# dmalyuta/explicit_hybrid_mpc

Measured on AMD Instinct MI355X. Metric: oracle LP solves/sec + final regions/sec, 4-state 2-input N=5 hybrid MPC, higher is better.
Workload: dtype f64

## Files before the change

explicit_hybrid_mpc_amd/csrc/ehm_dev.h:

```cpp
#pragma once

#include <hip/hip_runtime.h>
#include <stdint.h>

namespace ehm {

struct DevProblem {
    int n, m, p, n_u, n_delta;
    const double* Gt;
    const double* St;
    const double* w;
    const double* c;
    double eps_a, eps_r;
    const double* Wc2;
    int lda2, ncw2;
    const double* Wc4;
    int lda4, ncw4, tot4;
    int nd0, LE4;
    int wc_lds;
    const double* Wr3;
    int mpad3;
    const double* Hq;
    const double* Fq;
    const double* f0q;
// ... 78 lines not shown
        b1 = fmin(b1a, b1b);
        if (b1 < thr) return b1;
    }
    const int npairs = nr * (nr - 1) / 2;
    for (int t = lane; t < npairs; t += 64) {
        int a = 0, rem = t;
        while (rem >= nr - 1 - a) {
            rem -= nr - 1 - a;
            ++a;
        }
        const int c = a + 1 + rem;
        const double* fa = scr + a * na;
        const double* fc = scr + c * na;
        double m = -1e300;
        bool ok = true;
        for (int j = 0; j < na; ++j) {
            ok = ok && (fa[j] == fa[j]) && (fc[j] == fc[j]);
            m = fmax(m, fmin(fa[j], fc[j]));
        }
        for (int u = 0; u < na; ++u)
            for (int v = u + 1; v < na; ++v) {
                const double du = fa[u] - fc[u], dv = fa[v] - fc[v];
                if (du * dv < 0.0) {
                    const double den = du - dv;
                    double rc = __builtin_amdgcn_rcp(den);
                    rc = fma(rc, fma(-den, rc, 1.0), rc);
                    rc = fma(rc, fma(-den, rc, 1.0), rc);
                    const double sx = du * rc;
                    m = fmax(m, fma(sx, fa[v] - fa[u], fa[u]));
                }
            }
        if (ok) b = fmin(b, m);
    }
#define EHM_DPP_MIN_STEP(CTRL, RMASK)                                                          \
    {                                                                                          \
        const int lo = __builtin_amdgcn_update_dpp(__double2loint(1e300), __double2loint(b),   \
                                                   CTRL, RMASK, 0xf, false);                   \
        const int hi = __builtin_amdgcn_update_dpp(__double2hiint(1e300), __double2hiint(b),   \
                                                   CTRL, RMASK, 0xf, false);                   \
        b = fmin(b, __hiloint2double(hi, lo));                                                 \
    }
    EHM_DPP_MIN_STEP(0x111, 0xf)
    EHM_DPP_MIN_STEP(0x112, 0xf)
    EHM_DPP_MIN_STEP(0x114, 0xf)
    EHM_DPP_MIN_STEP(0x118, 0xf)
    EHM_DPP_MIN_STEP(0x142, 0xa)
    EHM_DPP_MIN_STEP(0x143, 0xc)
#undef EHM_DPP_MIN_STEP
    const int lo = __builtin_amdgcn_readlane(__double2loint(b), 63);
    const int hi = __builtin_amdgcn_readlane(__double2hiint(b), 63);
    return __hiloint2double(hi, lo);
}

struct DevCounters {
    unsigned long long lp_solves;
    unsigned long long ipm_iters;
    unsigned long long stalled;
    unsigned long long min_margin_bits;
    unsigned long long errors;
    unsigned long long slack_solves;
    unsigned long long slack_iters;
    unsigned long long cert_closed;
    unsigned long long wit_open;
    unsigned long long routed;
    unsigned long long wit_inherited;
    unsigned long long mid_shared;
    unsigned long long wit_table;
    unsigned long long prof[10];
    unsigned long long phase[24];
    unsigned int ticket;
    unsigned int ticket_pad;
};

__host__ __device__ inline int rec_off_vcost(int p) { return (p + 1) * p; }
__host__ __device__ inline int rec_off_vinput(int p) { return (p + 1) * p + (p + 1); }
__host__ __device__ inline int rec_doubles(int p, int n_u) {
    return (p + 1) * p + (p + 1) + (p + 1) * n_u;
}

enum { LP_POINT = 0, LP_FEAS = 1, LP_MIN_SIMPLEX = 2, LP_SLACK = 3, LP_FEAS_SIMPLEX = 4 };
enum { SX_MIN = 0, SX_SLACK = 1, SX_FEAS = 2 };

__host__ __device__ inline int lp_cols(const DevProblem& P, int kind) {
    switch (kind) {
        case LP_POINT: return P.n;
        case LP_FEAS: return P.n + 1;
        case LP_MIN_SIMPLEX: return P.n + P.p;
        case LP_FEAS_SIMPLEX: return P.n + P.p + 1;
        default: return P.n + P.p + 1;
    }
}
__host__ __device__ inline int lp_rows(const DevProblem& P, int kind) {
    switch (kind) {
        case LP_POINT: return P.m;
        case LP_FEAS: return P.m + 1;
        case LP_MIN_SIMPLEX: return P.m + P.p + 1;
        case LP_FEAS_SIMPLEX: return P.m + P.p + 2;
        default: return P.m + P.p + 3;
    }
}

__device__ inline void longest_edge(const double* R, int p, int& bi, int& bj) {
#pragma clang fp contract(off)
    double best = -1.0;
    bi = 0;
    bj = 1;
// ... 54 lines not shown
```

explicit_hybrid_mpc_amd/csrc/ehm_k2.h:

```cpp
#pragma once

#include <hip/hip_runtime.h>
#include <stdint.h>

#include "ehm_dev.h"

#ifndef EHM_K2_THREADS
#define EHM_K2_THREADS 768
#endif

#define K2_AUG_MIN 32
#define K2_HOT_GRAD 176
#define EHM_ROUTE_TOL 1e-6
#define EHM_REQUEUED 0x40000000

namespace ehm {

__host__ __device__ inline size_t k2_node_doubles(int p, int n_u) {
    const size_t nrec = ((size_t)rec_doubles(p, n_u) + 7) & ~(size_t)7;
    const size_t aug = (2 * (size_t)p * p > K2_AUG_MIN) ? 2 * (size_t)p * p : K2_AUG_MIN;
    return (nrec + aug + (size_t)p * p + 8 + 1) & ~(size_t)1;
}

__host__ __device__ inline int k2_stash_doubles(int p, int n_u) {
    return (n_u + 2 * p + 2 + 1) & ~1;
}

__host__ __device__ inline int lp_xbase(int m, int ne) {
    if (ne == 0) return m;
    const int r = m & 63;
    return (r != 0 && r + ne <= 64) ? m : ((m + 63) & ~63);
}
__host__ __device__ inline int lp_slots(int m, int ne) {
    return (lp_xbase(m, ne) + ne + 63) >> 6;
}

struct PersistCtl {
    int head;
    int pad0[31];
    int tail;
    int pad1[31];
    int pending;
    int pad2[31];
    int n_nodes;
    int pad3[31];
    int abort;
    int max_depth_seen;
    int truncated;
    int pad4;
    unsigned long long closed;
    unsigned long long splits;
    unsigned long long repl_closed, repl_splits, repl_solves;
    unsigned long long pushes;
};

struct PersistDeal {
    int pop_limit;
    int depth, rank, world;
    int mix;
    int keep;
    int check;
    int eager;
};

struct K2Gather {
// ... 54 lines not shown
```

explicit_hybrid_mpc_amd/csrc/ehm_persist.h:

```cpp
#ifndef EHM_PERSIST_H
#define EHM_PERSIST_H

#ifndef kx_persist
#error "kx_persist (the kernel's name) must be defined, and the namespace aliases kd / ke declared"
#endif

#define EHM_PERSIST_WATCHDOG_TICKS (60LL * 100000000LL)
#ifndef EHM_PERSIST_MIDFIRST
#define EHM_PERSIST_MIDFIRST 0
#endif
__global__ __launch_bounds__(EHM_K2_THREADS) void kx_persist(
    DevProblem P, DevTree T, int32_t* slots, int n_slots, PersistCtl* ctl, int node_cap,
    DevCounters* cnt, int wave_doubles, int sign_only, int max_depth, PersistDeal deal) {
    double* sm = reinterpret_cast<double*>(k2_smem);
    const int tid = threadIdx.x;
    const int lane0 = tid & 63;
    const int wave = __builtin_amdgcn_readfirstlane(tid >> 6);
    kd::Shared S;
    kd::carve_shared(S, sm, P);
    ke::Shared Se;
    ke::carve_shared(Se, sm, P);
#if EHM2_PROF
    S.gprof = cnt ? cnt->phase : nullptr;
    Se.gprof = cnt ? cnt->phase : nullptr;
#endif
    kd::NodeBuf nb;
    kd::carve_node(nb, sm + kd::shared_doubles(P) + (size_t)wave * wave_doubles, P.p, P.n_u);
    ke::NodeBuf nbe;
    ke::carve_node(nbe, sm + kd::shared_doubles(P) + (size_t)wave * wave_doubles, P.p, P.n_u);
    const int p = P.p, n_u = P.n_u;
    const int nrec = rec_doubles(p, n_u);
    kd::load_shared(P, 0, sm, tid, blockDim.x);
    __syncthreads();
    const long long t_start = wall_clock64();
    unsigned long long* wst = reinterpret_cast<unsigned long long*>(nb.aug);
    double* wmargin = nb.aug + 16;
    enum { W_SOLVES = 0, W_ITERS, W_STALLED, W_ERRORS, W_SLACK, W_SLACK_ITERS, W_CLOSED, W_SPLITS,
           W_DEPTH, W_TRUNC, W_CERT, W_WIT, W_ROUTED, W_RCLOSED, W_RSPLITS, W_RSOLVES,
           W_INH = 17, W_MT = 18, W_MTPARK = 19,
           W_TQ = 20, W_TMT = 21, W_TMID = 22, W_TSLK = 23, W_NMT = 24,
           W_WITT = 25, W_TPRE = 26, W_TPOST = 27, W_REQ = 28,
           W_EAGER = 29, W_PUSH = 30 };
    if (lane0 < 31 && lane0 != 16) wst[lane0] = 0ULL;
    if (lane0 == 0) *wmargin = 1e300;
    kd::wsync();
    int keep = -1;
    bool hot = false;
    int hot_dep = 0, hot_d = 0;
    bool hot_tested = false;
    const bool keep_child = deal.keep != 0;
    for (;;) {
        int id = -1;
        const bool is_hot = hot && keep >= 0;
        hot = false;
        if (keep >= 0) {
            id = keep;
            keep = -1;
        } else if (lane0 == 0) {
            const int idx = atomicAdd(&ctl->head, 1);
            if (idx < ((deal.pop_limit > 0 && deal.pop_limit < n_slots) ? deal.pop_limit
                                                                        : n_slots)) {
                long long t_q = 0;
                for (;;) {
                    id = __hip_atomic_load(&slots[idx], __ATOMIC_RELAXED, __HIP_MEMORY_SCOPE_AGENT);
                    if (id >= 0) break;
                    if (!t_q) t_q = wall_clock64();
                    if (__hip_atomic_load(&ctl->pending, __ATOMIC_RELAXED,
                                          __HIP_MEMORY_SCOPE_AGENT) <= 0 ||
                        __hip_atomic_load(&ctl->abort, __ATOMIC_RELAXED,
                                          __HIP_MEMORY_SCOPE_AGENT) != 0)
                        break;
                    if (wall_clock64() - t_start > EHM_PERSIST_WATCHDOG_TICKS) {
                        atomicMax(&ctl->abort, 3);
                        break;
                    }
                    __builtin_amdgcn_s_sleep(64);
                }
                if (t_q) wst[W_TQ] += (unsigned long long)(wall_clock64() - t_q);
            }
        }
        id = __builtin_amdgcn_readfirstlane(id);
        if (id < 0) break;
        const bool came_back = (id & EHM_REQUEUED) != 0;
        id &= ~EHM_REQUEUED;
        const long long t_pre = wall_clock64();
        const int lane = kd::pin(lane0);
        double* node = nb.rec;
        double* hgrad = nb.lp + K2_HOT_GRAD;
        const int ng = (p + 1) * p;
        int dep = hot_dep;
        if (!is_hot) {
            __builtin_amdgcn_fence(__ATOMIC_ACQUIRE, "agent");
            const double* rec = T.rec + (size_t)id * T.rec_stride;
            const double g_in = (T.grad && lane < ng) ? T.grad[(size_t)id * ng + lane] : 0.0;
#if EHM_PERSIST_MIDFIRST
            const double w_in = (T.wit && sign_only && lane < p + 2)
                ? T.wit[(size_t)id * (p + 2) + lane] : 0.0;
#endif
            dep = T.depth[id];
            for (int k = lane; k < nrec; k += 64) node[k] = rec[k];
            if (T.grad) {
                if (lane < ng) hgrad[lane] = g_in;
                for (int k = lane + 64; k < ng; k += 64) hgrad[k] = T.grad[(size_t)id * ng + k];
            }
#if EHM_PERSIST_MIDFIRST
            if (T.wit && sign_only && lane < p + 2)
                nb.rec[(size_t)wave_doubles - k2_stash_doubles(p, n_u) + n_u + p + lane] = w_in;
#endif
        }
        kd::wsync();
#if EHM_PERSIST_MIDFIRST
        auto lp_free_verdict = [&](const double* rec_, const double* g_, const double* w_,
                                   bool bound_done, double& tw, double& bnd) -> int {
            bool w_open = false;
            if (T.wit && sign_only) {
                const double* Vc = rec_ + rec_off_vcost(p);
                double vbw = 0.0;
                for (int q = 0; q <= p; ++q) vbw = fma(w_[1 + q], Vc[q], vbw);
                const double cw = w_[0];
                tw = fmin(vbw - cw - P.eps_a, vbw - (1.0 + P.eps_r) * cw);
                w_open = tw > EHM_ROUTE_TOL * (1.0 + fabs(vbw));
            }
            if (!(T.grad && sign_only) || bound_done || (w_open && !deal.check)) return w_open ? 1 : 0;
            const double thr = -EHM_ROUTE_TOL * (1.0 + fabs(rec_[rec_off_vcost(p)]));
            bnd = cut_bound(rec_, g_, p, P.eps_a, P.eps_r, lane, nb.lp, thr);
            if (w_open) {
                if (bnd < thr && lane == 0) wst[W_ERRORS] += 1;
                kd::wsync();
                return 1;
            }
            return bnd < thr ? 2 : 0;
        };
        bool inh_open = false;
        double inh_tw = 0.0;
        {
            double bnd = 0.0;
            const int verdict = lp_free_verdict(
                node, hgrad, nb.rec + (size_t)wave_doubles - k2_stash_doubles(p, n_u) + n_u + p,
                is_hot && hot_tested, inh_tw, bnd);
            inh_open = verdict == 1;
            if (verdict == 2) {
                if (lane == 0) {
                    const int dep0 = dep;
                    wst[W_CERT] += 1;
                    wst[W_CLOSED] += 1;
                    if (dep0 < deal.depth) wst[W_RCLOSED] += 1;
                    *wmargin = fmin(*wmargin, -bnd);
                    if ((unsigned long long)dep0 > wst[W_DEPTH]) wst[W_DEPTH] = (unsigned long long)dep0;
                    T.tstar[id] = bnd;
                    if (is_hot) T.flags[id] = 3;
                    else T.flags[id] |= 1;
                    atomicSub(&ctl->pending, 1);
                }
                kd::wsync();
                continue;
            }
        }
#else
        bool inh_open = false;
        double inh_tw = 0.0;
        if (T.grad && sign_only && inh_open && deal.check) {
            const double thr = -EHM_ROUTE_TOL * (1.0 + fabs(node[rec_off_vcost(p)]));
            const double bnd = cut_bound(node, hgrad, p, P.eps_a, P.eps_r, lane, nb.lp, thr);
            if (bnd < thr && lane == 0) wst[W_ERRORS] += 1;
            kd::wsync();
        }
        if (T.grad && sign_only && !inh_open) {
            const double thr = -EHM_ROUTE_TOL * (1.0 + fabs(node[rec_off_vcost(p)]));
            const double bnd = cut_bound(node, hgrad, p, P.eps_a, P.eps_r, lane, nb.lp, thr);
            if (bnd < thr) {
                if (lane == 0) {
                    const int dep0 = dep;
                    wst[W_CERT] += 1;
                    wst[W_CLOSED] += 1;
                    if (dep0 < deal.depth) wst[W_RCLOSED] += 1;
                    *wmargin = fmin(*wmargin, -bnd);
                    if ((unsigned long long)dep0 > wst[W_DEPTH]) wst[W_DEPTH] = (unsigned long long)dep0;
                    T.tstar[id] = bnd;
// ... 24 lines not shown
        bool decided = false;
        int c0_early = 0;
        bool alloc_early = false;
        if (T.wit && sign_only) {
            if (inh_open) {
                open = true;
                decided = true;
                have_wit = true;
                tst = inh_tw;
                margin = inh_tw;
                if (lane == 0) wst[W_INH] += 1;
            }
        }
        if (can_split) {
            longest_edge_wave(node, p, lane, bi, bj);
            if (lane < p) {
#pragma clang fp contract(off)
                mid[lane] = (node[bi * p + lane] + node[bj * p + lane]) / 2.0;
            }
            kd::wsync();
            if (T.mt.state) {
                unsigned int mt_i = 0u;
                int mt_slot = 0;
                const unsigned long long mt_tg = mt_tag(mid, p, T.mt.mask, &mt_i);
                if (lane == 0) {
                    wst[W_TPRE] += (unsigned long long)(wall_clock64() - t_pre);
                    long long waited = 0;
                    const bool may_requeue = decided && !came_back && deal.pop_limit <= 0 &&
                                             id < EHM_REQUEUED;
                    mt_res = mt_claim(T.mt, mt_tg, mt_i, t_start, EHM_PERSIST_WATCHDOG_TICKS,
                                      &mt_slot, &waited, may_requeue);
                    if (mt_res == MT_BUSY) {
                        const int t = atomicAdd(&ctl->tail, 1);
                        if (t < n_slots) {
                            __hip_atomic_store(&slots[t], id | EHM_REQUEUED, __ATOMIC_RELAXED,
                                               __HIP_MEMORY_SCOPE_AGENT);
                            wst[W_REQ] += 1;
                        } else {
                            mt_res = mt_claim(T.mt, mt_tg, mt_i, t_start,
                                              EHM_PERSIST_WATCHDOG_TICKS, &mt_slot, &waited);
                        }
                    }
                    if (waited) {
                        wst[W_TMT] += (unsigned long long)waited;
                        wst[W_NMT] += 1;
                    }
                }
                mt_res = __builtin_amdgcn_readfirstlane(mt_res);
                mt_slot = __builtin_amdgcn_readfirstlane(mt_slot);
                if (mt_res == MT_BUSY) {
                    kd::wsync();
                    continue;
                }
                if (deal.eager && decided) {
                    alloc_early = true;
                    if (lane == 0) c0_early = atomicAdd(&ctl->n_nodes, 2);
                }
                if (mt_res == MT_HIT) {
                    bool same = false;
                    const double ev = mt_read(T.mt, mt_slot, lane, mid, p, &same);
                    if (!same) {
                        mt_res = MT_NONE;
                    } else {
                        const int word = (int)__shfl(ev, 9);
                        Jm = __shfl(ev, 8);
                        mid_status = word & 0xff;
                        mid_conv = ((word >> 8) & 1) != 0;
                        mid_iters = 0;
                        if (lane >= 10 && lane < 10 + n_u) stash[lane - 10] = ev;
                        if (T.grad && lane >= 18 && lane < 18 + p) stash[st_g + lane - 18] = ev;
                        if (lane == 0) wst[W_MT] += 1;
                    }
                }
                if (lane == 0) wst[W_MTPARK] = (unsigned long long)mt_res |
                                               ((unsigned long long)mt_slot << 2);
            } else if (deal.eager && decided) {
                alloc_early = true;
                if (lane == 0) c0_early = atomicAdd(&ctl->n_nodes, 2);
            }
            if (mt_res != MT_HIT)
            {
            const long long t_mid = wall_clock64();
            ke::Wave Wm;
            ke::IpmResult rm;
            for (int attempt = 0; attempt < EHM2_ATTEMPTS; ++attempt) {
                double b[ke::SLOTS];
                const int ln = kd::pin(lane);
                ke::assemble_point(Se, Wm, nbe.lp, mid, false, b, ln, P, 0);
                rm = ke::ipm_solve(Se, Wm, b, ln, false, ke::step_fraction(attempt),
                                   T.grad ? nb.F : nullptr);
                its += rm.iters;
                if (rm.status == 0) break;
            }
#if EHM2_QUAD
            if (T.grad) ke::quad_grad_add(Wm, P, 0, mid, nb.F, lane);
#endif
            Jm = rm.obj;
            mid_status = rm.status;
            mid_conv = (rm.status == 0) && (rm.merit <= 1.0);
            mid_iters = its;
            if (lane < n_u) stash[lane] = Wm.xb[lane];
            if (lane == 0) wst[W_TMID] += (unsigned long long)(wall_clock64() - t_mid);
            }
            if (mt_res != MT_HIT && T.grad && lane < p) stash[st_g + lane] = nb.F[lane];
            kd::wsync();
            if (T.mt.state) {
                const unsigned long long park = wst[W_MTPARK];
                mt_res = (int)(park & 3ull);
                if (mt_res == MT_OWN) {
                    unsigned int mt_i = 0u;
                    const unsigned long long mt_tg = mt_tag(mid, p, T.mt.mask, &mt_i);
                    mt_publish(T.mt, (int)(park >> 2), mt_tg, lane, mid, p, Jm, mid_status,
                               mid_conv ? 1 : 0, mid_iters, stash, n_u,
                               T.grad ? stash + st_g : nullptr);
                }
            }
            if (sign_only && mid_conv && !decided) {
                const double* Vc = node + rec_off_vcost(p);
                const double vb = 0.5 * (Vc[bi] + Vc[bj]);
                const double tw = fmin(vb - Jm - P.eps_a, vb - (1.0 + P.eps_r) * Jm);
                if (tw > EHM_ROUTE_TOL * (1.0 + fabs(vb))) {
                    open = true;
                    decided = true;
                    tst = tw;
                    margin = tw;
                    if (lane == 0) wst[W_WIT] += 1;
                }
            }
        }
// ... 52 lines not shown
                    kd::wsync();
                }
            }
        }
#endif
        if (!decided) {
            const long long t_slk = wall_clock64();
            kd::Wave W;
            kd::IpmResult r;
            its = 0;
            for (int attempt = 0; attempt < EHM2_ATTEMPTS; ++attempt) {
                double b[kd::SLOTS];
                const int ln = kd::pin(lane);
                kd::assemble_simplex(S, W, nb, node, node + rec_off_vcost(p), SX_SLACK, P.eps_a,
                                     P.eps_r, b, ln, P, 0);
                r = kd::ipm_solve(S, W, b, ln, sign_only != 0, kd::step_fraction(attempt));
                its += r.iters;
                if (r.status == 0) break;
            }
            tst = -r.obj;
            open = (tst >= 0.0);
            margin = r.margin;
            const int slack_status = r.status;
#if !EHM2_QUAD
            if (T.wit && sign_only && open && slack_status == 0) {
                const int nz = S.n;
                double cz = 0.0, sb = 0.0;
                for (int q = 0; q < nz; ++q) cz = fma(S.cv[q], W.xb[kd::zcol(W, S, q)], cz);
                for (int q = 0; q < p; ++q) sb += W.xb[W.psi0 + q];
                kd::wsync();
                if (lane == 0) {
                    wit[0] = fma(EHM_WIT_REL, margin, cz);
                    wit[1] = 1.0 - sb;
                }
                if (lane < p) wit[2 + lane] = W.xb[W.psi0 + lane];
                have_wit = true;
                kd::wsync();
            }
#endif
            if (lane == 0) {
                wst[W_TSLK] += (unsigned long long)(wall_clock64() - t_slk);
                wst[W_SOLVES] += 1;
                if (dep < deal.depth) wst[W_RSOLVES] += 1;
                wst[W_ITERS] += (unsigned long long)its;
                wst[W_SLACK] += 1;
                wst[W_SLACK_ITERS] += (unsigned long long)its;
                if (slack_status != 0) {
                    wst[W_STALLED] += 1;
                    wst[W_ERRORS] += 1;
                    T.flags[id] |= 8;
                }
            }
        }
        if (lane == 0) {
            if (can_split) {
                if (mt_res != MT_HIT) {
                    wst[W_SOLVES] += 1;
                    if (dep < deal.depth) wst[W_RSOLVES] += 1;
                    wst[W_ITERS] += (unsigned long long)mid_iters;
                }
                if (mid_status != 0 && open) {
                    wst[W_STALLED] += 1;
                    wst[W_ERRORS] += 1;
                    T.flags[id] |= 16;
                }
            }
            *wmargin = fmin(*wmargin, margin);
            if (margin < EHM_ROUTE_TOL * (1.0 + fabs(node[rec_off_vcost(p)]))) wst[W_ROUTED] += 1;
            if ((unsigned long long)dep > wst[W_DEPTH]) wst[W_DEPTH] = (unsigned long long)dep;
            T.tstar[id] = tst;
            if (!open) {
                T.flags[id] |= 1;
                wst[W_CLOSED] += 1;
                if (dep < deal.depth) wst[W_RCLOSED] += 1;
            }
        }
        if (!open) {
            if (lane == 0) atomicSub(&ctl->pending, 1);
            kd::wsync();
            continue;
        }
        if (!can_split) {
            if (lane == 0) {
                wst[W_TRUNC] = 1;
                atomicSub(&ctl->pending, 1);
            }
            kd::wsync();
            continue;
        }
        const long long t_post = wall_clock64();
        const bool dealt = deal.world > 1 && dep + 1 == deal.depth;
        const bool fast = keep_child && !dealt;
        const bool eager = deal.eager != 0 && sign_only && T.grad && !dealt;
        const bool stage = fast || eager;
        double* hg0 = nb.lp + 256;
        double* cw0 = nb.lp + 328;
        double* c0rec = nb.lp + 340;
        const double gv0 = (T.grad && lane < ng) ? T.grad[(size_t)id * ng + lane] : 0.0;
        const int d = is_hot ? hot_d : T.didx[id];
        int c0 = c0_early;
        if (!alloc_early && lane == 0) c0 = atomicAdd(&ctl->n_nodes, 2);
        c0 = __builtin_amdgcn_readfirstlane(c0);
        if (c0 + 2 > node_cap) {
            if (lane == 0) {
                atomicMax(&ctl->abort, 1);
                atomicSub(&ctl->pending, 1);
            }
            break;
        }
        struct { double obj; } r = {Jm};
        if (T.grad) {
            const double* gp_ = T.grad + (size_t)id * ng;
            double* g0 = T.grad + (size_t)c0 * ng;
            for (int k = lane; k < ng; k += 64) {
                const double gv = (k < 64) ? gv0 : gp_[k];
                const double a0 = (k >= bi * p && k < bi * p + p) ? stash[st_g + k - bi * p] : gv;
                const double a1 = (k >= bj * p && k < bj * p + p) ? stash[st_g + k - bj * p] : gv;
                __hip_atomic_store(g0 + k, a0, __ATOMIC_RELAXED, __HIP_MEMORY_SCOPE_AGENT);
                __hip_atomic_store(g0 + ng + k, a1, __ATOMIC_RELAXED, __HIP_MEMORY_SCOPE_AGENT);
                if (stage) hgrad[k] = a1;
                if (eager) hg0[k] = a0;
            }
        }
        if (T.wit && lane < p + 2) {
            double* w0 = T.wit + (size_t)c0 * (p + 2);
            double v0 = 0.0, v1 = 0.0;
            if (have_wit) {
                witness_for_children(wit, node + rec_off_vcost(p), bi, bj, lane, v0, v1);
            }
            __hip_atomic_store(w0 + lane, v0, __ATOMIC_RELAXED, __HIP_MEMORY_SCOPE_AGENT);
            __hip_atomic_store(w0 + (p + 2) + lane, v1, __ATOMIC_RELAXED, __HIP_MEMORY_SCOPE_AGENT);
            kd::wsync();
            if (stage) wit[lane] = v1;
            if (eager) cw0[lane] = v0;
        }
        if (lane == 0) {
            wst[W_SPLITS] += 1;
            if (dep < deal.depth) wst[W_RSPLITS] += 1;
        }
        const double* xmid = stash;
#else
        kd::IpmResult r;
        int its = 0;
        {
            kd::Wave W;
            for (int attempt = 0; attempt < EHM2_ATTEMPTS; ++attempt) {
                double b[kd::SLOTS];
                const int ln = kd::pin(lane);
                kd::assemble_simplex(S, W, nb, node, node + rec_off_vcost(p), SX_SLACK, P.eps_a,
                                     P.eps_r, b, ln, P, 0);
                r = kd::ipm_solve(S, W, b, ln, sign_only != 0, kd::step_fraction(attempt));
                its += r.iters;
                if (r.status == 0) break;
            }
        }
        r.iters = its;
        const double tst = -r.obj;
        const bool open = (tst >= 0.0);
        if (lane == 0) {
            wst[W_SOLVES] += 1;
            if (dep < deal.depth) wst[W_RSOLVES] += 1;
            wst[W_ITERS] += (unsigned long long)r.iters;
            wst[W_SLACK] += 1;
            wst[W_SLACK_ITERS] += (unsigned long long)r.iters;
            if (r.status != 0) {
                wst[W_STALLED] += 1;
                wst[W_ERRORS] += 1;
                T.flags[id] |= 8;
            }
            *wmargin = fmin(*wmargin, r.margin);
            if (r.margin < EHM_ROUTE_TOL * (1.0 + fabs(node[rec_off_vcost(p)]))) wst[W_ROUTED] += 1;
            if ((unsigned long long)dep > wst[W_DEPTH]) wst[W_DEPTH] = (unsigned long long)dep;
            T.tstar[id] = tst;
            if (!open) {
                T.flags[id] |= 1;
                wst[W_CLOSED] += 1;
                if (dep < deal.depth) wst[W_RCLOSED] += 1;
            }
        }
        if (!open) {
            if (lane == 0) atomicSub(&ctl->pending, 1);
            kd::wsync();
            continue;
        }
        if (max_depth > 0 && dep >= max_depth) {
            if (lane == 0) {
                wst[W_TRUNC] = 1;
                atomicSub(&ctl->pending, 1);
            }
            kd::wsync();
            continue;
        }
        int c0 = 0;
        if (lane == 0) c0 = atomicAdd(&ctl->n_nodes, 2);
        c0 = __builtin_amdgcn_readfirstlane(c0);
        if (c0 + 2 > node_cap) {
            if (lane == 0) {
                atomicMax(&ctl->abort, 1);
                atomicSub(&ctl->pending, 1);
            }
            break;
        }
        double* mid = nb.th;
        int bi, bj;
        longest_edge_wave(node, p, lane, bi, bj);
        if (lane < p) {
#pragma clang fp contract(off)
            mid[lane] = (node[bi * p + lane] + node[bj * p + lane]) / 2.0;
        }
        kd::wsync();
        const int d = T.didx[id];
        ke::Wave W;
        ke::IpmResult re;
        its = 0;
        for (int attempt = 0; attempt < EHM2_ATTEMPTS; ++attempt) {
            double b[ke::SLOTS];
            const int ln = kd::pin(lane);
            ke::assemble_point(Se, W, nbe.lp, mid, false, b, ln, P, 0);
            re = ke::ipm_solve(Se, W, b, ln, false, ke::step_fraction(attempt),
                               T.grad ? nb.F : nullptr);
            its += re.iters;
            if (re.status == 0) break;
        }
        r.iters = its;
        r.status = re.status;
        r.obj = re.obj;
#if EHM2_QUAD
        if (T.grad) ke::quad_grad_add(W, P, 0, mid, nb.F, lane);
#endif
        if (T.grad) {
            const int ng = (p + 1) * p;
            const double* gp_ = T.grad + (size_t)id * ng;
            double* g0 = T.grad + (size_t)c0 * ng;
            for (int k = lane; k < ng; k += 64) {
                const double gv = gp_[k];
                const double a0 = (k >= bi * p && k < bi * p + p) ? nb.F[k - bi * p] : gv;
                const double a1 = (k >= bj * p && k < bj * p + p) ? nb.F[k - bj * p] : gv;
                __hip_atomic_store(g0 + k, a0, __ATOMIC_RELAXED, __HIP_MEMORY_SCOPE_AGENT);
                __hip_atomic_store(g0 + ng + k, a1, __ATOMIC_RELAXED, __HIP_MEMORY_SCOPE_AGENT);
            }
        }
        if (lane == 0) {
            wst[W_SOLVES] += 1;
            wst[W_ITERS] += (unsigned long long)r.iters;
            wst[W_SPLITS] += 1;
            if (dep < deal.depth) {
                wst[W_RSOLVES] += 1;
                wst[W_RSPLITS] += 1;
            }
            if (r.status != 0) {
                wst[W_STALLED] += 1;
                wst[W_ERRORS] += 1;
                T.flags[id] |= 16;
            }
        }
        const long long t_post = wall_clock64();
        const double* xmid = W.xb;
#endif
        double* rec0 = T.rec + (size_t)c0 * T.rec_stride;
        double* rec1 = rec0 + T.rec_stride;
        const int ov = rec_off_vcost(p), ou = rec_off_vinput(p);
        for (int k = lane; k < nrec; k += 64) {
            double v0 = node[k], v1 = node[k];
            if (k < ov) {
                if (k >= bi * p && k < bi * p + p) v0 = mid[k - bi * p];
                if (k >= bj * p && k < bj * p + p) v1 = mid[k - bj * p];
            } else if (k < ou) {
                if (k - ov == bi) v0 = r.obj;
                if (k - ov == bj) v1 = r.obj;
            } else {
                const int q = k - ou;
                if (q >= bi * n_u && q < bi * n_u + n_u) v0 = xmid[q - bi * n_u];
                if (q >= bj * n_u && q < bj * n_u + n_u) v1 = xmid[q - bj * n_u];
            }
            __hip_atomic_store(rec0 + k, v0, __ATOMIC_RELAXED, __HIP_MEMORY_SCOPE_AGENT);
            __hip_atomic_store(rec1 + k, v1, __ATOMIC_RELAXED, __HIP_MEMORY_SCOPE_AGENT);
#if EHM_PERSIST_MIDFIRST
            if (stage) node[k] = v1;
            if (eager) c0rec[k] = v0;
#endif
        }
        int closed0 = 0, closed1 = 0;
        double cbnd0 = 0.0, cbnd1 = 0.0;
#if EHM_PERSIST_MIDFIRST
        if (eager) {
            kd::wsync();
#pragma nounroll
            for (int c = 0; c < 2; ++c) {
                double tw_c = 0.0, bnd_c = 0.0;
                const int verdict = lp_free_verdict(c ? node : c0rec, c ? hgrad : hg0,
                                                    c ? wit : cw0, false, tw_c, bnd_c);
                if (verdict == 2) {
                    if (lane == 0) {
                        wst[W_CERT] += 1;
                        wst[W_CLOSED] += 1;
                        wst[W_EAGER] += 1;
                        if (dep + 1 < deal.depth) wst[W_RCLOSED] += 1;
                        *wmargin = fmin(*wmargin, -bnd_c);
                        if ((unsigned long long)(dep + 1) > wst[W_DEPTH])
                            wst[W_DEPTH] = (unsigned long long)(dep + 1);
                    }
                    if (c) { closed1 = 1; cbnd1 = bnd_c; }
                    else { closed0 = 1; cbnd0 = bnd_c; }
                }
                kd::wsync();
            }
        }
#endif
        int own0 = 1, own1 = 1;
        if (lane == 0) {
            T.left[id] = c0;
#define EHM_WT(ptr, val) __hip_atomic_store((ptr), (val), __ATOMIC_RELAXED, __HIP_MEMORY_SCOPE_AGENT)
            if (T.code) {
                const uint32_t pc = T.code[id];
                const uint32_t code0 = 2u * pc, code1 = 2u * pc + 1u;
                EHM_WT(&T.code[c0], code0);
                EHM_WT(&T.code[c0 + 1], code1);
                if (deal.world > 1 && dep + 1 == deal.depth) {
                    const uint32_t h0 = deal.mix ? ((code0 * 2654435761u) >> 12) : code0;
                    const uint32_t h1 = deal.mix ? ((code1 * 2654435761u) >> 12) : code1;
                    own0 = (int)(h0 % (uint32_t)deal.world) == deal.rank;
                    own1 = (int)(h1 % (uint32_t)deal.world) == deal.rank;
                }
            }
            EHM_WT(&T.left[c0], -1);
            EHM_WT(&T.left[c0 + 1], -1);
            EHM_WT(&T.didx[c0], d);
            EHM_WT(&T.didx[c0 + 1], d);
            EHM_WT(&T.depth[c0], dep + 1);
            EHM_WT(&T.depth[c0 + 1], dep + 1);
            EHM_WT(&T.flags[c0], (uint8_t)(closed0 ? 3 : own0 ? 2 : 6));
            EHM_WT(&T.flags[c0 + 1], (uint8_t)(closed1 ? 3 : own1 ? 2 : 6));
            EHM_WT(&T.tstar[c0], cbnd0);
            EHM_WT(&T.tstar[c0 + 1], cbnd1);
#undef EHM_WT
        }
        __builtin_amdgcn_fence(__ATOMIC_RELEASE, "workgroup");
        __builtin_amdgcn_s_waitcnt(0);
        int kept = -1;
        if (lane == 0) {
            const int need0 = own0 && !closed0, need1 = own1 && !closed1;
            const int nown = need0 + need1;
            int push0 = need0, push1 = need1;
            if (keep_child) {
                if (need1) { kept = c0 + 1; push1 = 0; }
                else if (need0) { kept = c0; push0 = 0; }
            }
            const int npush = push0 + push1;
            wst[W_PUSH] += (unsigned long long)npush;
            const int t = npush ? atomicAdd(&ctl->tail, npush) : 0;
            if (t + npush <= n_slots) {
                int at = t;
                if (push0)
                    __hip_atomic_store(&slots[at++], c0, __ATOMIC_RELAXED, __HIP_MEMORY_SCOPE_AGENT);
                if (push1)
                    __hip_atomic_store(&slots[at], c0 + 1, __ATOMIC_RELAXED,
                                       __HIP_MEMORY_SCOPE_AGENT);
                if (nown != 1) atomicAdd(&ctl->pending, nown - 1);
            } else {
                kept = -1;
                atomicMax(&ctl->abort, 1);
                atomicSub(&ctl->pending, 1);
            }
            wst[W_TPOST] += (unsigned long long)(wall_clock64() - t_post);
        }
        keep = __builtin_amdgcn_readfirstlane(kept);
#if EHM_PERSIST_MIDFIRST
        if (eager && keep == c0) {
            for (int k = lane; k < nrec; k += 64) node[k] = c0rec[k];
            for (int k = lane; k < ng; k += 64) hgrad[k] = hg0[k];
            if (T.wit && lane < p + 2) wit[lane] = cw0[lane];
        }
        hot = stage && keep >= 0;
        hot_tested = eager;
        hot_dep = dep + 1;
        hot_d = d;
#endif
        kd::wsync();
    }
    kd::wsync();
    if (lane0 == 0) {
        atomicAdd(&cnt->lp_solves, wst[W_SOLVES]);
        atomicAdd(&cnt->ipm_iters, wst[W_ITERS]);
        if (wst[W_STALLED]) atomicAdd(&cnt->stalled, wst[W_STALLED]);
        if (wst[W_ERRORS]) atomicAdd(&cnt->errors, wst[W_ERRORS]);
        atomicAdd(&cnt->slack_solves, wst[W_SLACK]);
        atomicAdd(&cnt->slack_iters, wst[W_SLACK_ITERS]);
        atomicMin(&cnt->min_margin_bits, (unsigned long long)__double_as_longlong(*wmargin));
        if (wst[W_CERT]) atomicAdd(&cnt->cert_closed, wst[W_CERT]);
        if (wst[W_WIT]) atomicAdd(&cnt->wit_open, wst[W_WIT]);
        if (wst[W_INH]) atomicAdd(&cnt->wit_inherited, wst[W_INH]);
        if (wst[W_MT]) atomicAdd(&cnt->mid_shared, wst[W_MT]);
        if (wst[W_WITT]) atomicAdd(&cnt->wit_table, wst[W_WITT]);
        atomicAdd(&cnt->prof[0], (unsigned long long)(wall_clock64() - t_start));
        if (wst[W_TQ]) atomicAdd(&cnt->prof[1], wst[W_TQ]);
        if (wst[W_TMT]) atomicAdd(&cnt->prof[2], wst[W_TMT]);
        if (wst[W_TMID]) atomicAdd(&cnt->prof[3], wst[W_TMID]);
        if (wst[W_TSLK]) atomicAdd(&cnt->prof[4], wst[W_TSLK]);
        if (wst[W_NMT]) atomicAdd(&cnt->prof[5], wst[W_NMT]);
        if (wst[W_TPRE]) atomicAdd(&cnt->prof[6], wst[W_TPRE]);
        if (wst[W_TPOST]) atomicAdd(&cnt->prof[7], wst[W_TPOST]);
        if (wst[W_REQ]) atomicAdd(&cnt->prof[8], wst[W_REQ]);
        if (wst[W_EAGER]) atomicAdd(&cnt->prof[9], wst[W_EAGER]);
        if (wst[W_PUSH]) atomicAdd(&ctl->pushes, wst[W_PUSH]);
        if (wst[W_ROUTED]) atomicAdd(&cnt->routed, wst[W_ROUTED]);
        atomicAdd(&ctl->closed, wst[W_CLOSED]);
        atomicAdd(&ctl->splits, wst[W_SPLITS]);
        if (wst[W_RCLOSED]) atomicAdd(&ctl->repl_closed, wst[W_RCLOSED]);
        if (wst[W_RSPLITS]) atomicAdd(&ctl->repl_splits, wst[W_RSPLITS]);
        if (wst[W_RSOLVES]) atomicAdd(&ctl->repl_solves, wst[W_RSOLVES]);
        atomicMax(&ctl->max_depth_seen, (int)wst[W_DEPTH]);
        if (wst[W_TRUNC]) atomicMax(&ctl->truncated, 1);
    }
}

#undef kx_persist

#endif
```

Measured before the change: 10.39 million.

## Specialize cut bound on p, allocate children early, stage child writes in LDS

Adds a template cut_bound_p specialized for p=2 and p=4, with unrolled loops and register-held rows, selected through a dispatch function. The child-node allocation atomic is now issued early for every decided or open split, not only in eager mode. Child record, gradient and witness data are built in LDS staging buffers and written to global memory after the child bound tests. The queue tail atomicAdd is also moved ahead of the release fence. The aim is to hide atomic latency and cut register and address overhead in the bound computation, at the cost of more LDS pressure and a new abort guard for large p.

```diff
diff --git a/explicit_hybrid_mpc_amd/csrc/ehm_dev.h b/explicit_hybrid_mpc_amd/csrc/ehm_dev.h
--- a/explicit_hybrid_mpc_amd/csrc/ehm_dev.h
+++ b/explicit_hybrid_mpc_amd/csrc/ehm_dev.h
@@ -154,6 +154,111 @@
     return __hiloint2double(hi, lo);
 }
 
+template <int P>
+__device__ inline double cut_bound_p(const double* node, const double* g, double eps_a,
+                                     double eps_r, int lane, double* scr, double thr = -1e301) {
+    constexpr int p = P, na = P + 1, nr = 2 * na;
+    const double* V = node + na * p;
+    for (int k = lane; k < na * na; k += 64) {
+        const int i = k / na, j = k - i * na;
+        double d = 0.0;
+#pragma unroll
+        for (int q = 0; q < p; ++q) d = fma(g[i * p + q], node[j * p + q] - node[i * p + q], d);
+        const double Li = V[i] + d;
+        scr[(2 * i) * na + j] = V[j] - Li - eps_a;
+        scr[(2 * i + 1) * na + j] = V[j] - (1.0 + eps_r) * Li;
+    }
+    __builtin_amdgcn_fence(__ATOMIC_ACQ_REL, "wavefront");
+    __builtin_amdgcn_wave_barrier();
+    double b = 1e300;
+    if (lane < nr) {
+        double m = -1e300;
+        bool ok = true;
+#pragma unroll
+        for (int j = 0; j < na; ++j) {
+            const double f = scr[lane * na + j];
+            ok = ok && (f == f);
+            m = fmax(m, f);
+        }
+        if (ok) b = m;
+    }
+    if (thr > -1e300) {
+        double b1 = b;
+#pragma unroll
+        for (int o = 8; o > 0; o >>= 1) b1 = fmin(b1, __shfl_xor(b1, o, 64));
+        const double b1a = __shfl(b1, 0, 64), b1b = __shfl(b1, 16, 64);
+        b1 = fmin(b1a, b1b);
+        if (b1 < thr) return b1;
+    }
+    constexpr int npairs = nr * (nr - 1) / 2;
+    for (int t = lane; t < npairs; t += 64) {
+        int a = 0, rem = t;
+#pragma unroll
+        for (int s = 0; s < nr - 2; ++s)
+            if (a == s && rem >= nr - 1 - s) {
+                rem -= nr - 1 - s;
+                a = s + 1;
+            }
+        const int c = a + 1 + rem;
+        double fa[na], fc[na];
+#pragma unroll
+        for (int j = 0; j < na; ++j) {
+            fa[j] = scr[a * na + j];
+            fc[j] = scr[c * na + j];
+        }
+        double m = -1e300;
+        bool ok = true;
+#pragma unroll
+        for (int j = 0; j < na; ++j) {
+            ok = ok && (fa[j] == fa[j]) && (fc[j] == fc[j]);
+            m = fmax(m, fmin(fa[j], fc[j]));
+        }
+#pragma unroll
+        for (int u = 0; u < na; ++u)
+#pragma unroll
+            for (int v = u + 1; v < na; ++v) {
+                const double du = fa[u] - fc[u], dv = fa[v] - fc[v];
+                if (du * dv < 0.0) {
+                    const double den = du - dv;
+                    double rc = __builtin_amdgcn_rcp(den);
+                    rc = fma(rc, fma(-den, rc, 1.0), rc);
+                    rc = fma(rc, fma(-den, rc, 1.0), rc);
+                    const double sx = du * rc;
+                    m = fmax(m, fma(sx, fa[v] - fa[u], fa[u]));
+                }
+            }
+        if (ok) b = fmin(b, m);
+    }
+#define EHM_DPP_MIN_STEP(CTRL, RMASK)                                                          \
+    {                                                                                          \
+        const int lo = __builtin_amdgcn_update_dpp(__double2loint(1e300), __double2loint(b),   \
+                                                   CTRL, RMASK, 0xf, false);                   \
+        const int hi = __builtin_amdgcn_update_dpp(__double2hiint(1e300), __double2hiint(b),   \
+                                                   CTRL, RMASK, 0xf, false);                   \
+        b = fmin(b, __hiloint2double(hi, lo));                                                 \
+    }
+    EHM_DPP_MIN_STEP(0x111, 0xf)
+    EHM_DPP_MIN_STEP(0x112, 0xf)
+    EHM_DPP_MIN_STEP(0x114, 0xf)
+    EHM_DPP_MIN_STEP(0x118, 0xf)
+    EHM_DPP_MIN_STEP(0x142, 0xa)
+    EHM_DPP_MIN_STEP(0x143, 0xc)
+#undef EHM_DPP_MIN_STEP
+    const int lo = __builtin_amdgcn_readlane(__double2loint(b), 63);
+    const int hi = __builtin_amdgcn_readlane(__double2hiint(b), 63);
+    return __hiloint2double(hi, lo);
+}
+
+__device__ inline double cut_bound_dispatch(const double* node, const double* g, int p,
+                                            double eps_a, double eps_r, int lane, double* scr,
+                                            double thr = -1e301) {
+    switch (p) {
+        case 2: return cut_bound_p<2>(node, g, eps_a, eps_r, lane, scr, thr);
+        case 4: return cut_bound_p<4>(node, g, eps_a, eps_r, lane, scr, thr);
+        default: return cut_bound(node, g, p, eps_a, eps_r, lane, scr, thr);
+    }
+}
+
 struct DevCounters {
     unsigned long long lp_solves;
     unsigned long long ipm_iters;
diff --git a/explicit_hybrid_mpc_amd/csrc/ehm_k2.h b/explicit_hybrid_mpc_amd/csrc/ehm_k2.h
--- a/explicit_hybrid_mpc_amd/csrc/ehm_k2.h
+++ b/explicit_hybrid_mpc_amd/csrc/ehm_k2.h
@@ -11,6 +11,12 @@
 
 #define K2_AUG_MIN 32
 #define K2_HOT_GRAD 176
+#define K2_C0_GRAD 256
+#define K2_C0_WIT 328
+#define K2_C0_REC 340
+static_assert(K2_HOT_GRAD >= 2 * 9 * 9 && K2_HOT_GRAD + 9 * 8 <= K2_C0_GRAD &&
+              K2_C0_GRAD + 9 * 8 <= K2_C0_WIT && K2_C0_WIT + 8 + 2 <= K2_C0_REC,
+              "LDS staging areas of the persistent kernel overlap at p = 8");
 #define EHM_ROUTE_TOL 1e-6
 #define EHM_REQUEUED 0x40000000
 
diff --git a/explicit_hybrid_mpc_amd/csrc/ehm_persist.h b/explicit_hybrid_mpc_amd/csrc/ehm_persist.h
--- a/explicit_hybrid_mpc_amd/csrc/ehm_persist.h
+++ b/explicit_hybrid_mpc_amd/csrc/ehm_persist.h
@@ -30,6 +30,13 @@
     ke::carve_node(nbe, sm + kd::shared_doubles(P) + (size_t)wave * wave_doubles, P.p, P.n_u);
     const int p = P.p, n_u = P.n_u;
     const int nrec = rec_doubles(p, n_u);
+#if EHM_PERSIST_MIDFIRST
+    if (p > 8 || K2_C0_REC + nrec > wave_doubles - (int)k2_node_doubles(p, n_u) -
+                                     k2_stash_doubles(p, n_u)) {
+        if (tid == 0) atomicMax(&ctl->abort, 1);
+        return;
+    }
+#endif
     kd::load_shared(P, 0, sm, tid, blockDim.x);
     __syncthreads();
     const long long t_start = wall_clock64();
@@ -123,7 +130,7 @@
             }
             if (!(T.grad && sign_only) || bound_done || (w_open && !deal.check)) return w_open ? 1 : 0;
             const double thr = -EHM_ROUTE_TOL * (1.0 + fabs(rec_[rec_off_vcost(p)]));
-            bnd = cut_bound(rec_, g_, p, P.eps_a, P.eps_r, lane, nb.lp, thr);
+            bnd = cut_bound_dispatch(rec_, g_, p, P.eps_a, P.eps_r, lane, nb.lp, thr);
             if (w_open) {
                 if (bnd < thr && lane == 0) wst[W_ERRORS] += 1;
                 kd::wsync();
@@ -254,7 +261,7 @@
                     kd::wsync();
                     continue;
                 }
-                if (deal.eager && decided) {
+                if (decided) {
                     alloc_early = true;
                     if (lane == 0) c0_early = atomicAdd(&ctl->n_nodes, 2);
                 }
@@ -276,7 +283,7 @@
                 }
                 if (lane == 0) wst[W_MTPARK] = (unsigned long long)mt_res |
                                                ((unsigned long long)mt_slot << 2);
-            } else if (deal.eager && decided) {
+            } else if (decided) {
                 alloc_early = true;
                 if (lane == 0) c0_early = atomicAdd(&ctl->n_nodes, 2);
             }
@@ -435,6 +442,10 @@
                 }
             }
         }
+        if (open && can_split && !alloc_early) {
+            alloc_early = true;
+            if (lane == 0) c0_early = atomicAdd(&ctl->n_nodes, 2);
+        }
         if (lane == 0) {
             if (can_split) {
                 if (mt_res != MT_HIT) {
@@ -475,173 +486,20 @@
         const bool dealt = deal.world > 1 && dep + 1 == deal.depth;
         const bool fast = keep_child && !dealt;
         const bool eager = deal.eager != 0 && sign_only && T.grad && !dealt;
-        const bool stage = fast || eager;
-        double* hg0 = nb.lp + 256;
-        double* cw0 = nb.lp + 328;
-        double* c0rec = nb.lp + 340;
+        double* hg0 = nb.lp + K2_C0_GRAD;
+        double* cw0 = nb.lp + K2_C0_WIT;
+        double* c0rec = nb.lp + K2_C0_REC;
         const double gv0 = (T.grad && lane < ng) ? T.grad[(size_t)id * ng + lane] : 0.0;
         const int d = is_hot ? hot_d : T.didx[id];
-        int c0 = c0_early;
-        if (!alloc_early && lane == 0) c0 = atomicAdd(&ctl->n_nodes, 2);
-        c0 = __builtin_amdgcn_readfirstlane(c0);
-        if (c0 + 2 > node_cap) {
-            if (lane == 0) {
-                atomicMax(&ctl->abort, 1);
-                atomicSub(&ctl->pending, 1);
-            }
-            break;
-        }
-        struct { double obj; } r = {Jm};
-        if (T.grad) {
-            const double* gp_ = T.grad + (size_t)id * ng;
-            double* g0 = T.grad + (size_t)c0 * ng;
-            for (int k = lane; k < ng; k += 64) {
-                const double gv = (k < 64) ? gv0 : gp_[k];
-                const double a0 = (k >= bi * p && k < bi * p + p) ? stash[st_g + k - bi * p] : gv;
-                const double a1 = (k >= bj * p && k < bj * p + p) ? stash[st_g + k - bj * p] : gv;
-                __hip_atomic_store(g0 + k, a0, __ATOMIC_RELAXED, __HIP_MEMORY_SCOPE_AGENT);
-                __hip_atomic_store(g0 + ng + k, a1, __ATOMIC_RELAXED, __HIP_MEMORY_SCOPE_AGENT);
-                if (stage) hgrad[k] = a1;
-                if (eager) hg0[k] = a0;
-            }
-        }
         if (T.wit && lane < p + 2) {
-            double* w0 = T.wit + (size_t)c0 * (p + 2);
             double v0 = 0.0, v1 = 0.0;
             if (have_wit) {
                 witness_for_children(wit, node + rec_off_vcost(p), bi, bj, lane, v0, v1);
             }
-            __hip_atomic_store(w0 + lane, v0, __ATOMIC_RELAXED, __HIP_MEMORY_SCOPE_AGENT);
-            __hip_atomic_store(w0 + (p + 2) + lane, v1, __ATOMIC_RELAXED, __HIP_MEMORY_SCOPE_AGENT);
             kd::wsync();
-            if (stage) wit[lane] = v1;
-            if (eager) cw0[lane] = v0;
-        }
-        if (lane == 0) {
-            wst[W_SPLITS] += 1;
-            if (dep < deal.depth) wst[W_RSPLITS] += 1;
-        }
-        const double* xmid = stash;
-#else
-        kd::IpmResult r;
-        int its = 0;
-        {
-            kd::Wave W;
-            for (int attempt = 0; attempt < EHM2_ATTEMPTS; ++attempt) {
-                double b[kd::SLOTS];
-                const int ln = kd::pin(lane);
-                kd::assemble_simplex(S, W, nb, node, node + rec_off_vcost(p), SX_SLACK, P.eps_a,
-                                     P.eps_r, b, ln, P, 0);
-                r = kd::ipm_solve(S, W, b, ln, sign_only != 0, kd::step_fraction(attempt));
-                its += r.iters;
-                if (r.status == 0) break;
-            }
-        }
-        r.iters = its;
-        const double tst = -r.obj;
-        const bool open = (tst >= 0.0);
-        if (lane == 0) {
-            wst[W_SOLVES] += 1;
-            if (dep < deal.depth) wst[W_RSOLVES] += 1;
-            wst[W_ITERS] += (unsigned long long)r.iters;
-            wst[W_SLACK] += 1;
-            wst[W_SLACK_ITERS] += (unsigned long long)r.iters;
-            if (r.status != 0) {
-                wst[W_STALLED] += 1;
-                wst[W_ERRORS] += 1;
-                T.flags[id] |= 8;
-            }
-            *wmargin = fmin(*wmargin, r.margin);
-            if (r.margin < EHM_ROUTE_TOL * (1.0 + fabs(node[rec_off_vcost(p)]))) wst[W_ROUTED] += 1;
-            if ((unsigned long long)dep > wst[W_DEPTH]) wst[W_DEPTH] = (unsigned long long)dep;
-            T.tstar[id] = tst;
-            if (!open) {
-                T.flags[id] |= 1;
-                wst[W_CLOSED] += 1;
-                if (dep < deal.depth) wst[W_RCLOSED] += 1;
-            }
-        }
-        if (!open) {
-            if (lane == 0) atomicSub(&ctl->pending, 1);
-            kd::wsync();
-            continue;
-        }
-        if (max_depth > 0 && dep >= max_depth) {
-            if (lane == 0) {
-                wst[W_TRUNC] = 1;
-                atomicSub(&ctl->pending, 1);
-            }
-            kd::wsync();
-            continue;
-        }
-        int c0 = 0;
-        if (lane == 0) c0 = atomicAdd(&ctl->n_nodes, 2);
-        c0 = __builtin_amdgcn_readfirstlane(c0);
-        if (c0 + 2 > node_cap) {
-            if (lane == 0) {
-                atomicMax(&ctl->abort, 1);
-                atomicSub(&ctl->pending, 1);
-            }
-            break;
-        }
-        double* mid = nb.th;
-        int bi, bj;
-        longest_edge_wave(node, p, lane, bi, bj);
-        if (lane < p) {
-#pragma clang fp contract(off)
-            mid[lane] = (node[bi * p + lane] + node[bj * p + lane]) / 2.0;
-        }
-        kd::wsync();
-        const int d = T.didx[id];
-        ke::Wave W;
-        ke::IpmResult re;
-        its = 0;
-        for (int attempt = 0; attempt < EHM2_ATTEMPTS; ++attempt) {
-            double b[ke::SLOTS];
-            const int ln = kd::pin(lane);
-            ke::assemble_point(Se, W, nbe.lp, mid, false, b, ln, P, 0);
-            re = ke::ipm_solve(Se, W, b, ln, false, ke::step_fraction(attempt),
-                               T.grad ? nb.F : nullptr);
-            its += re.iters;
-            if (re.status == 0) break;
-        }
-        r.iters = its;
-        r.status = re.status;
-        r.obj = re.obj;
-#if EHM2_QUAD
-        if (T.grad) ke::quad_grad_add(W, P, 0, mid, nb.F, lane);
-#endif
-        if (T.grad) {
-            const int ng = (p + 1) * p;
-            const double* gp_ = T.grad + (size_t)id * ng;
-            double* g0 = T.grad + (size_t)c0 * ng;
-            for (int k = lane; k < ng; k += 64) {
-                const double gv = gp_[k];
-                const double a0 = (k >= bi * p && k < bi * p + p) ? nb.F[k - bi * p] : gv;
-                const double a1 = (k >= bj * p && k < bj * p + p) ? nb.F[k - bj * p] : gv;
-                __hip_atomic_store(g0 + k, a0, __ATOMIC_RELAXED, __HIP_MEMORY_SCOPE_AGENT);
-                __hip_atomic_store(g0 + ng + k, a1, __ATOMIC_RELAXED, __HIP_MEMORY_SCOPE_AGENT);
-            }
-        }
-        if (lane == 0) {
-            wst[W_SOLVES] += 1;
-            wst[W_ITERS] += (unsigned long long)r.iters;
-            wst[W_SPLITS] += 1;
-            if (dep < deal.depth) {
-                wst[W_RSOLVES] += 1;
-                wst[W_RSPLITS] += 1;
-            }
-            if (r.status != 0) {
-                wst[W_STALLED] += 1;
-                wst[W_ERRORS] += 1;
-                T.flags[id] |= 16;
-            }
-        }
-        const long long t_post = wall_clock64();
-        const double* xmid = W.xb;
-#endif
-        double* rec0 = T.rec + (size_t)c0 * T.rec_stride;
-        double* rec1 = rec0 + T.rec_stride;
+            wit[lane] = v1;
+            cw0[lane] = v0;
+        }
         const int ov = rec_off_vcost(p), ou = rec_off_vinput(p);
         for (int k = lane; k < nrec; k += 64) {
             double v0 = node[k], v1 = node[k];
@@ -649,23 +507,28 @@
                 if (k >= bi * p && k < bi * p + p) v0 = mid[k - bi * p];
                 if (k >= bj * p && k < bj * p + p) v1 = mid[k - bj * p];
             } else if (k < ou) {
-                if (k - ov == bi) v0 = r.obj;
-                if (k - ov == bj) v1 = r.obj;
+                if (k - ov == bi) v0 = Jm;
+                if (k - ov == bj) v1 = Jm;
             } else {
                 const int q = k - ou;
-                if (q >= bi * n_u && q < bi * n_u + n_u) v0 = xmid[q - bi * n_u];
-                if (q >= bj * n_u && q < bj * n_u + n_u) v1 = xmid[q - bj * n_u];
-            }
-            __hip_atomic_store(rec0 + k, v0, __ATOMIC_RELAXED, __HIP_MEMORY_SCOPE_AGENT);
-            __hip_atomic_store(rec1 + k, v1, __ATOMIC_RELAXED, __HIP_MEMORY_SCOPE_AGENT);
-#if EHM_PERSIST_MIDFIRST
-            if (stage) node[k] = v1;
-            if (eager) c0rec[k] = v0;
-#endif
+                if (q >= bi * n_u && q < bi * n_u + n_u) v0 = stash[q - bi * n_u];
+                if (q >= bj * n_u && q < bj * n_u + n_u) v1 = stash[q - bj * n_u];
+            }
+            node[k] = v1;
+            c0rec[k] = v0;
+        }
+        if (T.grad) {
+            const double* gp_ = T.grad + (size_t)id * ng;
+            for (int k = lane; k < ng; k += 64) {
+                const double gv = (k < 64) ? gv0 : gp_[k];
+                const double a0 = (k >= bi * p && k < bi * p + p) ? stash[st_g + k - bi * p] : gv;
+                const double a1 = (k >= bj * p && k < bj * p + p) ? stash[st_g + k - bj * p] : gv;
+                hgrad[k] = a1;
+                hg0[k] = a0;
+            }
         }
         int closed0 = 0, closed1 = 0;
         double cbnd0 = 0.0, cbnd1 = 0.0;
-#if EHM_PERSIST_MIDFIRST
         if (eager) {
             kd::wsync();
 #pragma nounroll
@@ -689,8 +552,181 @@
                 kd::wsync();
             }
         }
+        const int c0 = __builtin_amdgcn_readfirstlane(c0_early);
+        if (c0 + 2 > node_cap) {
+            if (lane == 0) {
+                atomicMax(&ctl->abort, 1);
+                atomicSub(&ctl->pending, 1);
+            }
+            break;
+        }
+        if (lane == 0) {
+            wst[W_SPLITS] += 1;
+            if (dep < deal.depth) wst[W_RSPLITS] += 1;
+        }
+        if (T.grad) {
+            double* g0 = T.grad + (size_t)c0 * ng;
+            for (int k = lane; k < ng; k += 64) {
+                __hip_atomic_store(g0 + k, hg0[k], __ATOMIC_RELAXED, __HIP_MEMORY_SCOPE_AGENT);
+                __hip_atomic_store(g0 + ng + k, hgrad[k], __ATOMIC_RELAXED,
+                                   __HIP_MEMORY_SCOPE_AGENT);
+            }
+        }
+        if (T.wit && lane < p + 2) {
+            double* w0 = T.wit + (size_t)c0 * (p + 2);
+            __hip_atomic_store(w0 + lane, cw0[lane], __ATOMIC_RELAXED, __HIP_MEMORY_SCOPE_AGENT);
+            __hip_atomic_store(w0 + (p + 2) + lane, wit[lane], __ATOMIC_RELAXED,
+                               __HIP_MEMORY_SCOPE_AGENT);
+        }
+        {
+            double* rec0 = T.rec + (size_t)c0 * T.rec_stride;
+            double* rec1 = rec0 + T.rec_stride;
+            for (int k = lane; k < nrec; k += 64) {
+                __hip_atomic_store(rec0 + k, c0rec[k], __ATOMIC_RELAXED, __HIP_MEMORY_SCOPE_AGENT);
+                __hip_atomic_store(rec1 + k, node[k], __ATOMIC_RELAXED, __HIP_MEMORY_SCOPE_AGENT);
+            }
+        }
+#else
+        kd::IpmResult r;
+        int its = 0;
+        {
+            kd::Wave W;
+            for (int attempt = 0; attempt < EHM2_ATTEMPTS; ++attempt) {
+                double b[kd::SLOTS];
+                const int ln = kd::pin(lane);
+                kd::assemble_simplex(S, W, nb, node, node + rec_off_vcost(p), SX_SLACK, P.eps_a,
+                                     P.eps_r, b, ln, P, 0);
+                r = kd::ipm_solve(S, W, b, ln, sign_only != 0, kd::step_fraction(attempt));
+                its += r.iters;
+                if (r.status == 0) break;
+            }
+        }
+        r.iters = its;
+        const double tst = -r.obj;
+        const bool open = (tst >= 0.0);
+        if (lane == 0) {
+            wst[W_SOLVES] += 1;
+            if (dep < deal.depth) wst[W_RSOLVES] += 1;
+            wst[W_ITERS] += (unsigned long long)r.iters;
+            wst[W_SLACK] += 1;
+            wst[W_SLACK_ITERS] += (unsigned long long)r.iters;
+            if (r.status != 0) {
+                wst[W_STALLED] += 1;
+                wst[W_ERRORS] += 1;
+                T.flags[id] |= 8;
+            }
+            *wmargin = fmin(*wmargin, r.margin);
+            if (r.margin < EHM_ROUTE_TOL * (1.0 + fabs(node[rec_off_vcost(p)]))) wst[W_ROUTED] += 1;
+            if ((unsigned long long)dep > wst[W_DEPTH]) wst[W_DEPTH] = (unsigned long long)dep;
+            T.tstar[id] = tst;
+            if (!open) {
+                T.flags[id] |= 1;
+                wst[W_CLOSED] += 1;
+                if (dep < deal.depth) wst[W_RCLOSED] += 1;
+            }
+        }
+        if (!open) {
+            if (lane == 0) atomicSub(&ctl->pending, 1);
+            kd::wsync();
+            continue;
+        }
+        if (max_depth > 0 && dep >= max_depth) {
+            if (lane == 0) {
+                wst[W_TRUNC] = 1;
+                atomicSub(&ctl->pending, 1);
+            }
+            kd::wsync();
+            continue;
+        }
+        int c0 = 0;
+        if (lane == 0) c0 = atomicAdd(&ctl->n_nodes, 2);
+        c0 = __builtin_amdgcn_readfirstlane(c0);
+        if (c0 + 2 > node_cap) {
+            if (lane == 0) {
+                atomicMax(&ctl->abort, 1);
+                atomicSub(&ctl->pending, 1);
+            }
+            break;
+        }
+        double* mid = nb.th;
+        int bi, bj;
+        longest_edge_wave(node, p, lane, bi, bj);
+        if (lane < p) {
+#pragma clang fp contract(off)
+            mid[lane] = (node[bi * p + lane] + node[bj * p + lane]) / 2.0;
+        }
+        kd::wsync();
+        const int d = T.didx[id];
+        ke::Wave W;
+        ke::IpmResult re;
+        its = 0;
+        for (int attempt = 0; attempt < EHM2_ATTEMPTS; ++attempt) {
+            double b[ke::SLOTS];
+            const int ln = kd::pin(lane);
+            ke::assemble_point(Se, W, nbe.lp, mid, false, b, ln, P, 0);
+            re = ke::ipm_solve(Se, W, b, ln, false, ke::step_fraction(attempt),
+                               T.grad ? nb.F : nullptr);
+            its += re.iters;
+            if (re.status == 0) break;
+        }
+        r.iters = its;
+        r.status = re.status;
+        r.obj = re.obj;
+#if EHM2_QUAD
+        if (T.grad) ke::quad_grad_add(W, P, 0, mid, nb.F, lane);
+#endif
+        if (T.grad) {
+            const int ng = (p + 1) * p;
+            const double* gp_ = T.grad + (size_t)id * ng;
+            double* g0 = T.grad + (size_t)c0 * ng;
+            for (int k = lane; k < ng; k += 64) {
+                const double gv = gp_[k];
+                const double a0 = (k >= bi * p && k < bi * p + p) ? nb.F[k - bi * p] : gv;
+                const double a1 = (k >= bj * p && k < bj * p + p) ? nb.F[k - bj * p] : gv;
+                __hip_atomic_store(g0 + k, a0, __ATOMIC_RELAXED, __HIP_MEMORY_SCOPE_AGENT);
+                __hip_atomic_store(g0 + ng + k, a1, __ATOMIC_RELAXED, __HIP_MEMORY_SCOPE_AGENT);
+            }
+        }
+        if (lane == 0) {
+            wst[W_SOLVES] += 1;
+            wst[W_ITERS] += (unsigned long long)r.iters;
+            wst[W_SPLITS] += 1;
+            if (dep < deal.depth) {
+                wst[W_RSOLVES] += 1;
+                wst[W_RSPLITS] += 1;
+            }
+            if (r.status != 0) {
+                wst[W_STALLED] += 1;
+                wst[W_ERRORS] += 1;
+                T.flags[id] |= 16;
+            }
+        }
+        const long long t_post = wall_clock64();
+        const double* xmid = W.xb;
+        double* rec0 = T.rec + (size_t)c0 * T.rec_stride;
+        double* rec1 = rec0 + T.rec_stride;
+        const int ov = rec_off_vcost(p), ou = rec_off_vinput(p);
+        for (int k = lane; k < nrec; k += 64) {
+            double v0 = node[k], v1 = node[k];
+            if (k < ov) {
+                if (k >= bi * p && k < bi * p + p) v0 = mid[k - bi * p];
+                if (k >= bj * p && k < bj * p + p) v1 = mid[k - bj * p];
+            } else if (k < ou) {
+                if (k - ov == bi) v0 = r.obj;
+                if (k - ov == bj) v1 = r.obj;
+            } else {
+                const int q = k - ou;
+                if (q >= bi * n_u && q < bi * n_u + n_u) v0 = xmid[q - bi * n_u];
+                if (q >= bj * n_u && q < bj * n_u + n_u) v1 = xmid[q - bj * n_u];
+            }
+            __hip_atomic_store(rec0 + k, v0, __ATOMIC_RELAXED, __HIP_MEMORY_SCOPE_AGENT);
+            __hip_atomic_store(rec1 + k, v1, __ATOMIC_RELAXED, __HIP_MEMORY_SCOPE_AGENT);
+        }
+        const int closed0 = 0, closed1 = 0;
+        const double cbnd0 = 0.0, cbnd1 = 0.0;
 #endif
         int own0 = 1, own1 = 1;
+        int kept = -1, need0 = 0, need1 = 0, push0 = 0, push1 = 0, tail_at = 0;
         if (lane == 0) {
             T.left[id] = c0;
 #define EHM_WT(ptr, val) __hip_atomic_store((ptr), (val), __ATOMIC_RELAXED, __HIP_MEMORY_SCOPE_AGENT)
@@ -717,23 +753,24 @@
             EHM_WT(&T.tstar[c0], cbnd0);
             EHM_WT(&T.tstar[c0 + 1], cbnd1);
 #undef EHM_WT
-        }
-        __builtin_amdgcn_fence(__ATOMIC_RELEASE, "workgroup");
-        __builtin_amdgcn_s_waitcnt(0);
-        int kept = -1;
-        if (lane == 0) {
-            const int need0 = own0 && !closed0, need1 = own1 && !closed1;
-            const int nown = need0 + need1;
-            int push0 = need0, push1 = need1;
+            need0 = own0 && !closed0;
+            need1 = own1 && !closed1;
+            push0 = need0;
+            push1 = need1;
             if (keep_child) {
                 if (need1) { kept = c0 + 1; push1 = 0; }
                 else if (need0) { kept = c0; push0 = 0; }
             }
             const int npush = push0 + push1;
             wst[W_PUSH] += (unsigned long long)npush;
-            const int t = npush ? atomicAdd(&ctl->tail, npush) : 0;
-            if (t + npush <= n_slots) {
-                int at = t;
+            if (npush) tail_at = atomicAdd(&ctl->tail, npush);
+        }
+        __builtin_amdgcn_fence(__ATOMIC_RELEASE, "workgroup");
+        __builtin_amdgcn_s_waitcnt(0);
+        if (lane == 0) {
+            const int nown = need0 + need1, npush = push0 + push1;
+            if (tail_at + npush <= n_slots) {
+                int at = tail_at;
                 if (push0)
                     __hip_atomic_store(&slots[at++], c0, __ATOMIC_RELAXED, __HIP_MEMORY_SCOPE_AGENT);
                 if (push1)
@@ -754,7 +791,7 @@
             for (int k = lane; k < ng; k += 64) hgrad[k] = hg0[k];
             if (T.wit && lane < p + 2) wit[lane] = cw0[lane];
         }
-        hot = stage && keep >= 0;
+        hot = (fast || eager) && keep >= 0;
         hot_tested = eager;
         hot_dep = dep + 1;
         hot_d = d;
```

New measurement: 10.53 million (median of 6 runs). +1.3%, better.
